# dovidio/jepsen-etcd-demo

Measured on AMD Instinct MI355X. Metric: history ops linearizability-checked/sec (whole node), higher is better.
Workload: dtype u32

## Files before the change

jepsen-etcd-demo_amd/csrc/device_api.hip:

```cpp

#include <dlfcn.h>

#include <atomic>
#include <chrono>
#include <cstring>
#include <functional>
#include <string>
#include <thread>

#include "device_ctx.hpp"

using namespace lcx;

const Rccl *lcx::rccl() {
    static Rccl r;
    static std::once_flag once;
    std::call_once(once, [] {
        void *h = nullptr;
        Dl_info info;
        if (dladdr((void *)&hipStreamCreateWithFlags, &info) && info.dli_fname) {
            std::string dir = info.dli_fname;
            dir = dir.substr(0, dir.find_last_of('/') + 1);
            for (const char *name : {"librccl.so.1", "librccl.so"})
                if (!h) h = dlopen((dir + name).c_str(), RTLD_NOW | RTLD_LOCAL);
// ... 892 lines not shown
        st->total_ms = std::chrono::duration<double, std::milli>(std::chrono::steady_clock::now() - s.t0).count();
        st->lds_keys = c->hctl[2];
        st->wgl_keys = c->hctl[2];
        st->wgl_steps = c->hctl[1];
        st->events = c->hctl[1];
        st->probes = c->hctl[0];
        st->wgl_spilled = ws.wgl_spilled;
    }
    return LC_OK;
}

static int ensure_spec_ws(const Step &s) {
    Dev *c = s.c;
    Lane &L = *s.L;
    LCCHK(grow_dev(c, L.spec_ws, L.spec_ws_words, lcd::spec_ws_words(s.K, s.p.segs)));
    LCCHK(grow_dev(c, L.spec_fin, L.spec_fin_words, s.p.exact ? lcd::spec_fin_words(s.K, s.p.segs) : (size_t)0));
    const int64_t rr_had = L.spec_rr_cap;
    LCCHK(grow_dev(c, L.spec_rr, L.spec_rr_cap, s.K + 2));
    if (L.spec_rr_cap != rr_had) HIPCHK(hipMemsetAsync(L.spec_rr, 0, 2 * sizeof(int32_t), s.q));
    return LC_OK;
}

static int t0_args(Step &s, lcd::Args *a0) {
    Dev *c = s.c;
    if (s.p.t0_step && c->ticket_live && !s.p.competition) {
        s.ticket_base = c->ticket_next;
    } else {
        LCCHK(zero_control(c, s.q));
    }
    c->ticket_live = false;
    if (s.a.n_final && s.K > 0) HIPCHK(hipMemsetAsync(s.a.n_final, 0, (size_t)s.K * 4, s.q));
    const Lists l = lists_of(c);
    *a0 = s.a;
    a0->order = s.d->order; a0->n_order = (int32_t)s.K; a0->n_in = nullptr; a0->ticket = c->counters + 8;
    a0->spill = l.spill0; a0->n_spill = l.n_spill0; a0->wide = l.wide; a0->n_wide = l.n_wide;
    a0->deep = l.spill2; a0->n_deep = l.n_spill2;
    a0->lat_ws = nullptr;
    return LC_OK;
}

static int args_slot(Lane &L, const lcd::Args &a0, lcd::Args **dargs) {
    int aslot = -1;
    for (int q = 0; q < Lane::ARGS_RING && aslot < 0; ++q)
        if (L.args_ok[q] && std::memcmp(L.hargs + q, &a0, sizeof a0) == 0) aslot = q;
    if (aslot < 0) {
        aslot = (int)(L.args_next++ % Lane::ARGS_RING);
        HIPCHK(hipEventSynchronize(L.args_ev[aslot]));
        std::memcpy(L.hargs + aslot, &a0, sizeof a0);
        HIPCHK(hipMemcpyAsync(L.dargs + aslot, L.hargs + aslot, sizeof(lcd::Args), hipMemcpyHostToDevice, L.stream));
        HIPCHK(hipEventRecord(L.args_ev[aslot], L.stream));
        L.args_ok[aslot] = true;
    }
    *dargs = L.dargs + aslot;
    return LC_OK;
}

static lcd::SegArgs seg_args(const Step &s, int grid) {
    Dev *c = s.c;
    const DevBatch *d = s.d;
    const lcd::Args &a = s.a;
    lcd::SegArgs sa{};
    sa.ev_off = d->ev_off; sa.events = d->events; sa.trans = d->trans; sa.key_error = d->key_error;
    sa.n_trans = (uint32_t)d->n_trans; sa.n_keys = (int32_t)s.K; sa.max_seg = lcd::SEG_MAX;
    const double per_key = std::max(1.0, 2.0 * grid / (double)s.K);
    sa.seg_len = (uint32_t)std::max<double>(64.0, (double)d->n_events / (double)s.K / per_key);
    if (c->o->seg_len > 0) sa.seg_len = (uint32_t)c->o->seg_len;
    sa.seg_cnt = c->seg_cnt; sa.seg_end = c->seg_end; sa.seg_out = c->seg_out; sa.seg0_fev = c->seg0_fev;
    sa.work = c->seg_work; sa.rerun = c->seg_rerun; sa.rerun_init = c->seg_rerun_init; sa.ctl = c->seg_ctl;
    sa.err = a.err; sa.valid = a.valid; sa.fail_event = a.fail_event; sa.cause = a.cause;
    sa.rec = a.rec;
    sa.strict = a.strict;
    sa.err_base = a.err_base;
    return sa;
}

static lcd::SpecLaunch spec_launch(const Step &s) {
    Dev *c = s.c;
    const lc_opts &o = *c->o;
    lcd::SpecLaunch l{};
    l.segs = s.p.segs;
    l.ws = s.L->spec_ws; l.rr = s.L->spec_rr; l.parity = s.L->spec_parity;
    l.ck1 = o.spec_ck ? ((uint32_t)o.spec_ck & 0xFFFFu) - 1u : 32u;
    l.ck2 = o.spec_ck ? ((uint32_t)o.spec_ck >> 16) - 1u : 120u;
    l.rerun_grid = c->cu_count;
    l.validate_blocks = s.p.spec_vblocks;
    l.events16 = s.p.ev16 ? s.d->events16 : nullptr;
    l.cost_cuts = (o.path_flags & LC_PATH_SPEC_COST) != 0;
    l.prio = !(o.path_flags & LC_PATH_SPEC_NOPRIO) && !(s.lu && s.lu->overlap);
    l.vfirst = s.p.spec_vfirst;
    l.fin = s.p.exact ? s.L->spec_fin : nullptr;
    l.stage = !(o.path_flags & LC_PATH_SPEC_NOSTAGE);
    return l;
}

static int launch_register_tier(Step &s, const lcd::Args &a0, const lcd::Args *dargs) {
    Dev *c = s.c;
    const lc::StepPlan &p = s.p;
    const int64_t K = s.K;
    if (p.side_validate) {
        HIPCHK(hipEventRecord(c->vin, c->stream));
        HIPCHK(hipStreamWaitEvent(c->stream1, c->vin, 0));
        lcd::Args av = s.a;
        av.n_order = (int32_t)K;
        HIPCHK(lcd::launch_validate(av, c->stream1, p.gen_validate));
        HIPCHK(hipEventRecord(c->vdone, c->stream1));
    }
    if (p.split) {
        const int grid = c->cu_count * 12;
        HIPCHK(hipMemsetAsync(c->seg_ctl, 0, 4 * sizeof(int32_t), c->stream));
        HIPCHK(lcd::launch_segments(seg_args(s, grid), grid, c->stream));
        if (!p.async) HIPCHK(hipEventRecord(c->et0, c->stream));
    } else if (p.spec) {
        HIPCHK(lcd::launch_spec(a0, dargs, spec_launch(s), s.q));
        s.L->spec_parity ^= 1;
        if (!p.async) HIPCHK(hipEventRecord(c->et0, s.q));
    } else if (K > 0 && !s.d->table) {
        HIPCHK(lcd::launch_t0(a0, dargs, p.g0, p.t0_wide, c->stream, s.ticket_base));
        if (!p.async) HIPCHK(hipEventRecord(c->et0, c->stream));
    } else if (K > 0) {
        HIPCHK(hipEventRecord(c->et0, c->stream));
    }
    if (p.side_validate) HIPCHK(hipStreamWaitEvent(c->stream, c->vdone, 0));
    return LC_OK;
}

static void keep_ticket(const Step &s) {
    s.c->ticket_next = (s.p.split || s.p.spec) ? s.ticket_base : s.ticket_base + (uint32_t)s.K + (uint32_t)s.p.g0;
    s.c->ticket_live = true;
}

static int finish_async(const Step &s, lc_stats *st, bool *enqueued) {
    Dev *c = s.c;
    if (s.lu && s.lu->dst) {
        if (s.lu->after) HIPCHK(hipStreamWaitEvent(s.q, s.lu->after, 0));
        HIPCHK(hipMemcpyAsync(s.lu->dst, s.L->rec, s.lu->n * 8, hipMemcpyDeviceToHost, s.q));
    }
    HIPCHK(hipEventRecord(c->ring[c->async_seq % 4], s.q));
    if (s.lu && s.lu->overlap) {
        ++c->run_n;
        c->lane1_live |= s.lu->lane == 1;
    }
    c->ea1_pending = true;
    ++c->async_seq;
    ++c->n_async;
    keep_ticket(s);
    if (st) {
        *st = lc_stats{};
        st->t0_path = s.p.t0_path;
        st->ev_word_bytes = s.p.ev_word_bytes;
    }
    if (enqueued) *enqueued = true;
    return LC_OK;
}

static int run_set_tiers(const Step &s) {
    Dev *c = s.c;
    const Lists l = lists_of(c);
    lcd::Args a1 = s.a;
    a1.order = l.spill0; a1.n_order = 0; a1.n_in = l.n_spill0; a1.ticket = c->counters + 9;
    if (s.d->table) { a1.order = s.d->order; a1.n_order = (int32_t)s.K; a1.n_in = nullptr; }
    a1.spill = l.spill1; a1.n_spill = l.n_spill1; a1.wide = l.wide; a1.n_wide = l.n_wide;
    int g1 = (int)std::min<int64_t>(s.K, (int64_t)c->cu_count * 7);
    HIPCHK(lcd::launch_t1(a1, g1, c->stream));
    lcd::Args a2 = s.a;
    a2.order = l.spill1; a2.n_order = 0; a2.n_in = l.n_spill1; a2.ticket = c->counters + 10;
    a2.spill = l.spill2; a2.n_spill = l.n_spill2; a2.wide = l.wide; a2.n_wide = l.n_wide;
    HIPCHK(lcd::launch_t2(a2, c->cu_count, c->stream));
    return LC_OK;
}

static int read_t0_step(const Step &s) {
// ... 435 lines not shown
```

jepsen-etcd-demo_amd/csrc/device_spec.hip:

```cpp

#include "lattice_core.hpp"
#include "lattice_validate.hpp"

namespace lcd {


constexpr uint32_t SPEC_NONE = 0xFFFFFFFFu;
constexpr uint32_t SPEC_MIN_LEN = 128;
constexpr uint32_t SPEC_MAX_PEND = 6;

template <class EvT>
__device__ __forceinline__ int32_t spec_net(EvT evp, uint32_t b, uint32_t e) {
    constexpr uint32_t G = 8;
    const uint32_t lane = lane_id();
    int32_t cnt = 0;
    for (uint32_t gb = b; gb < e; gb += 64 * G) {
        uint32_t wg[G];
#pragma unroll
        for (uint32_t g = 0; g < G; ++g) {
            const uint32_t j = gb + 64 * g + lane;
            wg[g] = j < e ? evp[j] : 0u;
        }
#pragma unroll
        for (uint32_t g = 0; g < G; ++g) {
// ... 523 lines not shown
__device__ unsigned long long lc_spec_stamps[4096 * 8 * 12];
extern "C" int lc_debug_spec_stamps(unsigned long long *host, int n) {
    return (int)hipMemcpyFromSymbol(host, HIP_SYMBOL(lc_spec_stamps), (size_t)n * 8 * 12 * 8, 0, hipMemcpyDeviceToHost);
}
#define SPEC_STAMP(s, k, v) \
    if (lane == 0 && blk < 4096 && (s) < 8) lc_spec_stamps[((size_t)blk * 8 + (s)) * 12 + (k)] = (v);
#else
#define SPEC_STAMP(s, k, v)
#endif

template <int S, bool E16>
constexpr uint32_t spec_ev_lds() { return (E16 && S > 2) ? (S >= 8 && SPEC_NCK > 2 ? 3072u : 4096u) : 0u; }

#ifndef LC_SPEC2_WAVES
#define LC_SPEC2_WAVES 8
#endif
template <int S, bool E16, bool EX = false>
__global__ __launch_bounds__(64 * S, (S == 2 ? LC_SPEC2_WAVES : S == 8 ? LC_SPEC8_WAVES : 1)) void k_spec(T0Args a) {
#define KA t0k()
    constexpr uint32_t EVC = spec_ev_lds<S, E16>();
    __shared__ uint16_t s_ev[EVC ? EVC : 1];
    __shared__ uint32_t s_end[S][64];
    __shared__ uint32_t s_ck[S][SPEC_NCK][64];
    __shared__ uint32_t s_pend[S][8];
    __shared__ uint64_t s_map[S];
    __shared__ int32_t s_ck_e[S][SPEC_NCK];
    __shared__ int32_t s_cut[S], s_segend[S];
    __shared__ int32_t s_top[S];
    __shared__ int32_t s_ver[S], s_vfev[S];
    __shared__ int32_t s_net[S];
    __shared__ int32_t s_cand[S], s_ncand[S];
    __shared__ int32_t s_prdy[S], s_done[S];
    __shared__ uint32_t s_vx[S][2];
    constexpr bool MEETC = LC_SPEC_MEET && !EX;
    __shared__ int32_t s_meet[MEETC ? S : 1][SPEC_MEET_N];
    constexpr int NWS = spec_lds_ws<S>();
    __shared__ uint32_t s_ws[NWS ? NWS * 3 * T0_RMEM * 64 : 1];
    __shared__ int32_t s_ws_busy[NWS ? NWS : 1];
    const uint32_t lane = lane_id(), wv = uni((uint32_t)threadIdx.x >> 6);
    const uint32_t nb = gridDim.x - (uint32_t)KA.n_order;
    const bool vfirst = (KA.flags & T0_SPEC_VFIRST) != 0;
    const uint32_t blk = vfirst ? blockIdx.x - nb : blockIdx.x;
    if (vfirst ? blockIdx.x < nb : blockIdx.x >= (uint32_t)KA.n_order) {
        const uint32_t vb = vfirst ? blockIdx.x : blockIdx.x - (uint32_t)KA.n_order;
        for (int64_t k = (int64_t)vb * S + wv; k < KA.n_order; k += (int64_t)nb * S) {
            if (EVC > 0 && !(KA.flags & T0_SPEC_NOSTAGE) && KA.ev_off[k + 1] - KA.ev_off[k] <= EVC) continue;
            validate_key<false, E16>(a, k);
        }
        return;
    }
    const int32_t key = (int32_t)uni((uint32_t)KA.order[blk]);
    uint32_t *ws = KA.lat_ws + ((size_t)blk * S + wv) * (3 * T0_RMEM * 64);
    const uint64_t eb = KA.ev_off[key];
    const uint32_t nev = (uint32_t)(KA.ev_off[key + 1] - eb);
    uint32_t n_lds = 0;
    if constexpr (EVC > 0) {
        if (!(KA.flags & T0_SPEC_NOSTAGE)) {
            n_lds = nev < EVC ? nev : EVC;
            const uint16_t *g = KA.events16 + eb;
            for (uint32_t base = 0; base < n_lds; base += 64u * S * 8u) {
                uint16_t v[8];
#pragma unroll
                for (uint32_t q = 0; q < 8; ++q) {
                    const uint32_t j = base + q * 64u * S + threadIdx.x;
                    v[q] = j < n_lds ? g[j] : (uint16_t)0;
                }
#pragma unroll
                for (uint32_t q = 0; q < 8; ++q) {
                    const uint32_t j = base + q * 64u * S + threadIdx.x;
                    if (j < n_lds) s_ev[j] = v[q];
                }
            }
        }
    }
    using EvK = typename std::conditional<(EVC > 0), EvStaged, EvSrc<E16>>::type;
    EvK evp;
    if constexpr (EVC > 0) evp = EvStaged{(LdsU16 *)s_ev, KA.events16 + eb, n_lds};
    else evp = ev_src<E16>(KA) + eb;
    const uint32_t tb = KA.trans_off ? KA.trans_off[key] : 0u;
    const uint32_t ntr = KA.n_trans > tb ? KA.n_trans - tb : 0u;
    const uint32_t *const trp = KA.trans + (ntr ? tb : 0u);
    const uint32_t nstates = KA.trans_off ? (KA.key_states ? KA.key_states[key] : 0xFFFFu) : KA.shared_states;
    const uint32_t width = KA.key_width ? KA.key_width[key] : 0xFFu;
    const bool plain = (KA.key_error && KA.key_error[key]) || nstates > T0_MAX_STATES || nstates == 0 ||
                       width > T0_MAX_WIDTH || KA.init_state >= T0_MAX_STATES || nev < 2 * SPEC_MIN_LEN;
    const uint32_t eff = plain ? 1u : min((uint32_t)S, nev / SPEC_MIN_LEN);
    const uint32_t topmask = nstates >= 32 ? ~0u : (1u << nstates) - 1u;

    if (threadIdx.x < NWS) s_ws_busy[threadIdx.x] = 0;
    if (MEETC && threadIdx.x < S * SPEC_MEET_N) s_meet[threadIdx.x / SPEC_MEET_N][threadIdx.x % SPEC_MEET_N] = -1;
    __syncthreads();
    bool self_val = false;
    uint32_t vc0 = 0, vc1 = 0;
    if constexpr (EVC > 0) {
        self_val = (KA.flags & T0_STRICT) && !(KA.flags & T0_SPEC_NOSTAGE) && n_lds == nev &&
                   !(KA.key_error && KA.key_error[key]);
        const uint32_t nch = (nev + 63u) / 64u;
        vc0 = nch * wv / S;
        vc1 = nch * (wv + 1u) / S;
        if (self_val) {
            uint32_t x0 = 0, x1 = 0;
            for (uint32_t ch = vc0; ch < vc1; ++ch) {
                const uint32_t j = ch * 64u + lane;
                if (j < nev) {
                    const uint32_t sl = LC_EV_SLOT(LC_EV16_WIDE(s_ev[j]));
                    x0 ^= sl < 32u ? 1u << sl : 0u;
                    x1 ^= (sl >= 32u && sl < 64u) ? 1u << (sl - 32u) : 0u;
                }
            }
            x0 = uni(__ockl_wfred_xor_u32(x0));
            x1 = uni(__ockl_wfred_xor_u32(x1));
            if (lane == 0) { s_vx[wv][0] = x0; s_vx[wv][1] = x1; }
        }
    }
    if (wv == 0) {
        for (uint32_t s = 0; s < (uint32_t)S; ++s) { SPEC_STAMP(s, 0, __builtin_amdgcn_s_memtime()) }
    }
    const bool cost = (KA.flags & T0_SPEC_COST) != 0;
    if (!plain && !cost) {
        for (uint32_t p = wv; p + 1 < eff; p += S) {
            const uint32_t t0 = (uint32_t)((uint64_t)nev * p / eff), t1 = (uint32_t)((uint64_t)nev * (p + 1) / eff);
            const int32_t d = spec_net(evp, t0, t1);
            if (lane == 0) s_net[p] = d;
        }
    }
    __syncthreads();
    if constexpr (EVC > 0) {
        if (self_val) {
            const uint32_t vns = KA.trans_off ? (KA.key_states ? KA.key_states[key] : 0u) : KA.shared_states;
            uint32_t pend[2] = {0u, 0u};
            for (uint32_t q = 0; q < wv; ++q) { pend[0] ^= uni(s_vx[q][0]); pend[1] ^= uni(s_vx[q][1]); }
            int32_t why = 0;
            for (uint32_t ch = vc0; ch < vc1 && !why; ++ch) {
                const uint32_t j = ch * 64u + lane;
                const bool in = j < nev;
                const uint32_t w = in ? LC_EV16_WIDE(s_ev[j]) : 0u;
                why = validate_chunk<false, 2>(w, in, trp, ntr, vns, 64u, pend);
            }
            if (why && lane == 0) {
                atomicOr(&KA.err[0], why);
                atomicMax(&KA.err[1], KA.err_base + key + 1);
            }
        }
    }
    if (!plain && !cost) {
        for (uint32_t s = wv; s < eff; s += S) {
            if (s == 0) continue;
            int32_t pend = 0;
            for (uint32_t q = 0; q < s; ++q) pend += uni(s_net[q]);
            const uint32_t t = (uint32_t)((uint64_t)nev * s / eff);
            const uint32_t w = t + lane < nev ? evp[t + lane] : 0u;
            uint32_t n2 = 0;
            const uint32_t c2 = spec_cut_at(w, nev, t, pend, n2);
            if (lane == 0) {
                s_cand[s] = c2 == SPEC_NONE ? -1 : (int32_t)c2;
                s_ncand[s] = (int32_t)n2;
            }
        }
    }
    if (!plain && cost && wv < eff) {
        uint32_t pos_v;
        int32_t pend_v;
        spec_targets_cost(evp, nev, eff, pos_v, pend_v);
        for (uint32_t s = wv; s < eff; s += S) {
            if (s == 0) continue;
            const uint32_t t = uni(__builtin_amdgcn_readlane(pos_v, s));
            const uint32_t w = t + lane < nev ? evp[t + lane] : 0u;
            uint32_t n2 = 0;
            const uint32_t c2 = spec_cut_at(w, nev, t, uni(__builtin_amdgcn_readlane(pend_v, s)), n2);
// ... 46 lines not shown
            if (s == 0) {
                st.W0 = lane == 0 ? 1u << KA.init_state : 0u;
            } else {
                words = spec_pending(evp, cut, n0, np);
                spec_setup(st, words, np, trp, ntr);
                st.W0 = lane < (1u << np) ? topmask : 0u;
            }
            if (lane < 6) s_pend[s][lane] = words;
            if (lane == 6) s_pend[s][6] = np;
            const bool lost = s != 0 && np != n0;
            if (lost && lane == 0) s_top[s] = -3;
            spec_publish(&s_prdy[s]);
            uint32_t fev = 0;
            uint32_t *const sv = EX ? KA.spec_fin + ((size_t)blk * S + s) * 2 * SPEC_SAVE_WORDS : nullptr;
            const int r = lost ? 6
                               : spec_walk<0, NWS, EvK, EX>(evp, trp, ntr, cut, end, st, ws, s_ws, s_ws_busy,
                                                                   s_ck[s], s_ck_e[s], KA.spec_ck1, KA.spec_ck2,
                                                                   fev, !(KA.flags & T0_SPEC_NOPRIO), sv, nullptr,
                                                                   (MEETC && s != 0) ? s_meet[s] : nullptr);
            s_end[s][lane] = st.W0;
            uint64_t map = 0;
            for (uint32_t q = 0; q < 6; ++q) {
                const uint32_t sl = __builtin_amdgcn_readlane(st.slot_v, q);
                if ((st.live >> q) & 1u) map |= (uint64_t)(0x80u | sl) << (8 * q);
            }
            SPEC_STAMP(s, 2, __builtin_amdgcn_s_memtime())
            top_s = r == 1 ? (int32_t)fev : r == 3 ? -2 : r == 6 ? -3 : -1;
            if (lane == 0) {
                s_map[s] = map;
                s_top[s] = top_s;
            }
            spec_publish(&s_done[s]);
        }
        uint32_t v = s + 1;
        while (v < eff && uni(s_cut[v]) < 0) ++v;
        if (kept && top_s == -1 && v < eff) {
            SPEC_STAMP(v, 3, __builtin_amdgcn_s_memtime())
            int32_t ver = 3, vfev = -1;
            uint32_t fev = 0;
            if (spec_wait(&s_prdy[v]) && spec_load(&s_top[v]) != -3) {
                const uint32_t cut = (uint32_t)uni(s_cut[v]), end = (uint32_t)uni(s_segend[v]);
                const uint32_t np = uni(s_pend[v][6]);
                SpecState st{};
                spec_setup(st, lane < 6 ? s_pend[v][lane] : 0u, np, trp, ntr);
                const uint64_t map = uni(s_map[s]);
                uint32_t src = 0;
                for (uint32_t j = 0; j < np; ++j) {
                    const uint32_t sl = __builtin_amdgcn_readlane(st.slot_v, j);
                    uint32_t at = 31;
                    for (uint32_t q = 0; q < 6; ++q)
                        if (((map >> (8 * q)) & 0xFFu) == (0x80u | sl)) at = q;
                    src |= ((lane >> j) & 1u) << at;
                }
                const uint32_t E = (uint32_t)__shfl((int)s_end[s][lane], (int)(src & 63u));
                st.W0 = lane < (1u << np) ? E : 0u;
                uint32_t *const sv =
                    EX ? KA.spec_fin + ((size_t)blk * S + v) * 2 * SPEC_SAVE_WORDS + SPEC_SAVE_WORDS : nullptr;
                const int r = spec_walk<1, NWS, EvK, EX>(evp, trp, ntr, cut, end, st, ws, s_ws, s_ws_busy,
                                                                s_ck[v], s_ck_e[v], 0, 0, fev, false, sv,
                                                                &s_done[v], MEETC ? s_meet[v] : nullptr);
                bool last = true;
                for (uint32_t q = v + 1; q < eff; ++q) last = last && uni(s_cut[q]) < 0;
                if (r == 4) ver = 1;
                else if (r == 1) { ver = 2; vfev = (int32_t)fev; }
                else if (r == 3) ver = 6;
                else if (r == 5) ver = 3;
                else if (last) ver = 5;
                else if (spec_wait(&s_done[v])) ver = (st.n <= 6 && !__any(st.W0 != s_end[v][lane])) ? 1 : 3;
            }
            SPEC_STAMP(v, 7, ((unsigned long long)ver << 32) | (fev - (uint32_t)uni(s_cut[v])))
            SPEC_STAMP(v, 4, __builtin_amdgcn_s_memtime())
            if (lane == 0) {
                s_ver[v] = ver;
                s_vfev[v] = vfev;
            }
        }
    }
    __syncthreads();
    if (wv == 0) {
        for (uint32_t s = 0; s < (uint32_t)S; ++s) { SPEC_STAMP(s, 5, __builtin_amdgcn_s_memtime()) }
    }
    if (wv == 0) {
        const Args &f = *KA.full;
        bool rerun = plain, bad = false;
        int32_t fv = -1;
        uint32_t fin_run = 0;
        if (!plain) {
            for (uint32_t s = 0; s < eff && fv < 0 && !rerun && !bad; ++s) {
                if (uni(s_cut[s]) < 0) continue;
                const int32_t top = uni(s_top[s]);
                if (top == -2) { bad = true; break; }
                if (top == -3) { rerun = true; break; }
                fin_run = 2 * s;
                if (s == 0) { fv = top; continue; }
                const int32_t ver = uni(s_ver[s]);
                if (ver == 1) fv = top;
                else if (ver == 2) { fv = uni(s_vfev[s]); fin_run = 2 * s + 1; }
                else if (ver == 5) fin_run = 2 * s + 1;
                else if (ver == 6) bad = true;
                else rerun = true;
            }
        }
        int kr = K_DONE;
        if (rerun) {
            if (lane == 0) KA.spec_rr[atomicAdd(KA.spec_nrr, 1)] = key;
        } else if (bad) kr = K_SPILL;
        else if (fv >= 0) finish_key(f, key, LC_INVALID, LC_CAUSE_NONLIN, fv, 0, 0, (uint64_t)fv + 1u);
        else finish_key(f, key, LC_VALID, LC_CAUSE_NONE, -1, 0, 0, nev);
        if constexpr (EX) {
            if (!rerun && !bad) {
                uint32_t *const sv = KA.spec_fin + ((size_t)blk * S * 2 + fin_run) * SPEC_SAVE_WORDS;
                const LatMem fm{sv, sv, sv};
                write_final_mem(f, key, fm, lane, sv[T0_RMEM * 64 + lane], uni(sv[(T0_RMEM + 1) * 64]));
            }
        }
        if (kr == K_SPILL) {
            if (KA.flags & T0_STRICT) {
                t0_malformed(KA, key, LC_BATCH_E_FIT);
                finish_key(f, key, LC_UNKNOWN, LC_CAUSE_ERROR, -1, 0, 0, 0);
            } else {
                const bool deep = f.deep && KA.key_width && KA.key_width[key] > LC_DIRECT_T3_WIDTH;
                push_list(deep ? f.deep : f.spill, deep ? f.n_deep : f.n_spill, key, f.list_cap);
            }
        }
    }
}
#undef KA

constexpr int SPEC_RERUN_WAVES = 4;
template <bool E16, bool EX = false>
__global__ __launch_bounds__(64 * SPEC_RERUN_WAVES) void k_spec_rerun(T0Args a) {
    __shared__ uint32_t ws_all[SPEC_RERUN_WAVES][3 * T0_RMEM * 64];
    uint32_t *const ws = ws_all[threadIdx.x >> 6];
    const int32_t n = *a.spec_nrr;
    if (blockIdx.x == 0 && threadIdx.x == 0) *a.spec_nrr_next = 0;
    for (int32_t w = blockIdx.x * SPEC_RERUN_WAVES + (int32_t)(threadIdx.x >> 6); w < n;
         w += gridDim.x * SPEC_RERUN_WAVES) {
        const int32_t key = a.spec_rr[w];
        const int kr = lattice_key<T0_RSMALL, !EX, E16>(a, key, ws);
        if (kr == K_SPILL) t0_spill(a, key);
    }
}

#ifdef LC_T0_COUNT_SWEEPS
int spec_sweep_hist(unsigned long long *host) {
    return (int)hipMemcpyFromSymbol(host, HIP_SYMBOL(lc_sweep_hist), sizeof(lc_sweep_hist), 0, hipMemcpyDeviceToHost);
}
#endif

size_t spec_ws_words(int64_t n_keys, int segs) { return (size_t)std::max<int64_t>(n_keys, 1) * segs * lat_ws_words(); }

size_t spec_fin_words(int64_t n_keys, int segs) {
    return (size_t)std::max<int64_t>(n_keys, 1) * segs * 2 * SPEC_SAVE_WORDS;
}
hipError_t launch_spec(const Args &a, const Args *a_dev, const SpecLaunch &l, hipStream_t s) {
    const int segs = l.segs;
    const uint16_t *const events16 = l.events16;
    uint32_t *const fin = l.fin;
    T0Args t = make_t0(a, a_dev);
    t.events16 = events16;
    if (l.cost_cuts) t.flags |= T0_SPEC_COST;
    if (!l.stage) t.flags |= T0_SPEC_NOSTAGE;
    if (l.vfirst && l.validate_blocks > 0) t.flags |= T0_SPEC_VFIRST;
    if (!l.prio) t.flags |= T0_SPEC_NOPRIO;
    t.lat_ws = l.ws;
    t.spec_ck1 = l.ck1;
    t.spec_ck2 = l.ck2;
    t.spec_nrr = l.rr + (l.parity & 1);
    t.spec_nrr_next = l.rr + ((l.parity & 1) ^ 1);
    t.spec_rr = l.rr + 2;
    t.spec_fin = fin;
    const dim3 grid((unsigned)std::max(1, a.n_order + std::max(0, l.validate_blocks)));
    const dim3 rgrid((unsigned)std::max(1, std::min((a.n_order + SPEC_RERUN_WAVES - 1) / SPEC_RERUN_WAVES, l.rerun_grid)));
#define LC_SPEC_L(SS, E, X) hipLaunchKernelGGL((k_spec<SS, E, X>), grid, dim3(64 * SS), 0, s, t)
#define LC_SPEC_ALL(E)                                      \
    if (fin) {                                              \
        if (segs >= 8) LC_SPEC_L(8, E, true);               \
        else if (segs >= 4) LC_SPEC_L(4, E, true);          \
        else LC_SPEC_L(2, E, true);                         \
    } else if (segs >= 8) LC_SPEC_L(8, E, false);           \
    else if (segs >= 6) LC_SPEC_L(6, E, false);             \
    else if (segs >= 4) LC_SPEC_L(4, E, false);             \
    else if (segs >= 3) LC_SPEC_L(3, E, false);             \
    else LC_SPEC_L(2, E, false);
    if (events16) { LC_SPEC_ALL(true) } else { LC_SPEC_ALL(false) }
#undef LC_SPEC_ALL
#undef LC_SPEC_L
    hipError_t e = hipGetLastError();
    if (e != hipSuccess) return e;
    if (events16) {
        if (fin) hipLaunchKernelGGL((k_spec_rerun<true, true>), rgrid, dim3(64 * SPEC_RERUN_WAVES), 0, s, t);
        else hipLaunchKernelGGL((k_spec_rerun<true, false>), rgrid, dim3(64 * SPEC_RERUN_WAVES), 0, s, t);
    } else {
        if (fin) hipLaunchKernelGGL((k_spec_rerun<false, true>), rgrid, dim3(64 * SPEC_RERUN_WAVES), 0, s, t);
        else hipLaunchKernelGGL((k_spec_rerun<false, false>), rgrid, dim3(64 * SPEC_RERUN_WAVES), 0, s, t);
    }
    return hipGetLastError();
}

}
```

jepsen-etcd-demo_amd/csrc/lattice_core.hpp:

```cpp
#pragma once

#include <hip/hip_runtime.h>

#include <type_traits>

#include <algorithm>
#include <cstdint>

#include "../../include/lincheck.h"
#include "device_common.hpp"
#include "device_search.hpp"
#include "stream_plan.hpp"

extern "C" __device__ uint32_t __ockl_wfred_add_u32(uint32_t);
extern "C" __device__ int32_t __ockl_wfred_add_i32(int32_t);
extern "C" __device__ uint32_t __ockl_wfred_min_u32(uint32_t);
extern "C" __device__ uint32_t __ockl_wfred_xor_u32(uint32_t);

namespace lcd {

constexpr int T0_RSMALL = 4, T0_RBIG = 16;
constexpr int T0_RMEM = 16;
#ifndef LC_T0_MAX_WIDTH
#define LC_T0_MAX_WIDTH 10
// ... 904 lines not shown
    uint32_t W0 = W[0];
    bool dirty = true;
    [[maybe_unused]] bool dense_first = false;
    if constexpr (RESUME) {
        if constexpr (FAST) dirty = rs->dirty;
        dense_first = n >= 7;
    }
    for (uint32_t phase = 0; phase <= nev && e < lim; ++phase) {
        while (e < lim && !(RESUME && dense_first)) {
            T0_PROF_BEGIN
            const uint32_t evi = __builtin_amdgcn_readlane(ev, i);
            const uint32_t slot = LC_EV_SLOT(evi);
            if (!(evi & LC_EV_OK_BIT)) {
                if (n == 6) break;
                if (n >= T0_MAX_WIDTH || slot >= 64) {
                    status = 3;
                } else {
                    const Xfer x{(uint32_t)__builtin_amdgcn_readlane(xc.k, i),
                                 (uint32_t)__builtin_amdgcn_readlane(xc.cap, i),
                                 (uint32_t)__builtin_amdgcn_readlane(xc.b, i)};
                    const uint32_t idx = (uint32_t)__builtin_ctz(~live);
                    slot_v = setl(slot_v, idx, slot);
                    k_v = setl(k_v, idx, x.k);
                    cap_v = setl(cap_v, idx, x.cap);
                    b_v = setl(b_v, idx, x.b);
                    if constexpr (TAG) m_v = setl(m_v, idx, (uint32_t)__builtin_amdgcn_readlane(xc.m, i));
                    dense_v = setl(dense_v, slot, idx);
                    live |= 1u << idx;
                    ++n;
                    dirty = true;
                }
            } else {
                const uint32_t p = __builtin_amdgcn_readlane(dense_v, slot & 63u);
                uint32_t nSn = 0;
                int r;
                if constexpr (FAST && RM == T0_RSMALL) {
                    const uint32_t top = 32u - (uint32_t)__builtin_clz(live);
                    if (top >= 6) r = ok_lane_closed<6, TAG>(W0, p, live, k_v, cap_v, b_v, lane, lm, dirty, m_v);
                    else if (top == 5) r = ok_lane_closed<5, TAG>(W0, p, live, k_v, cap_v, b_v, lane, lm, dirty, m_v);
                    else r = ok_lane_closed<4, TAG>(W0, p, live, k_v, cap_v, b_v, lane, lm, dirty, m_v);
                    dirty = false;
                    k_v = setl(k_v, p, 0u);
                } else {
                const uint32_t pk = __builtin_amdgcn_readlane(k_v, p), pc = __builtin_amdgcn_readlane(cap_v, p),
                               pb = __builtin_amdgcn_readlane(b_v, p);
                k_v = setl(k_v, p, 0u);
                const uint32_t top = 32u - (uint32_t)__builtin_clz(live);
                if (RM == T0_RBIG || top >= 6)
                    r = ok_lane<6>(W0, p, live, k_v, cap_v, b_v, pk, pc, pb, lane, lm, budget, count, probes, nSn,
                                   want_peak);
                else if (top == 5)
                    r = ok_lane<5>(W0, p, live, k_v, cap_v, b_v, pk, pc, pb, lane, lm, budget, count, probes, nSn,
                                   want_peak);
                else
                    r = ok_lane<4>(W0, p, live, k_v, cap_v, b_v, pk, pc, pb, lane, lm, budget, count, probes, nSn,
                                   want_peak);
                }
                live = r ? live : live & ~(1u << p);
                n = r ? n : n - 1;
                peak = nSn > peak ? nSn : peak;
                status = r;
                fev = e;
            }
            T0_PROF_END(evi)
            lim = status ? 0u : lim;
            advance();
        }
        if (e >= lim) break;
        if (!(RESUME && dense_first)) {
            W[0] = W0;
#pragma unroll
            for (int k = 1; k < RM; ++k) W[k] = 0u;
        }
        if constexpr (RESUME) dense_first = false;
        while (e < lim) {
            T0_PROF_BEGIN
            const uint32_t evi = __builtin_amdgcn_readlane(ev, i);
            const uint32_t slot = LC_EV_SLOT(evi);
            if (!(evi & LC_EV_OK_BIT)) {
                if (n >= T0_MAX_WIDTH || slot >= 64) {
                    status = 3;
                } else {
                    if (RM < 16 && n == 8) {
#pragma unroll
                        for (int k = 0; k < T0_RMEM; ++k) m.W[k * 64 + lane] = k < RM ? W[k < RM ? k : 0] : 0u;
                        in_mem = true;
                    }
                    const Xfer x{(uint32_t)__builtin_amdgcn_readlane(xc.k, i),
                                 (uint32_t)__builtin_amdgcn_readlane(xc.cap, i),
                                 (uint32_t)__builtin_amdgcn_readlane(xc.b, i)};
                    const uint32_t idx = n;
                    slot_v = setl(slot_v, idx, slot);
                    k_v = setl(k_v, idx, x.k);
                    cap_v = setl(cap_v, idx, x.cap);
                    b_v = setl(b_v, idx, x.b);
                    if constexpr (TAG) m_v = setl(m_v, idx, (uint32_t)__builtin_amdgcn_readlane(xc.m, i));
                    dense_v = setl(dense_v, slot, idx);
                    live |= 1u << idx;
                    ++n;
                }
            } else {
                const uint32_t p = __builtin_amdgcn_readlane(dense_v, slot & 63u);
                uint32_t nSn = 0;
                int r;
                if (n == 7)
                    r = ok_reg<2, RM, TAG>(W, p, k_v, cap_v, b_v, lane, budget, count, probes, nSn, want_peak, m_v);
                else if (n == 8)
                    r = ok_reg<4, RM, TAG>(W, p, k_v, cap_v, b_v, lane, budget, count, probes, nSn, want_peak, m_v);
                else if constexpr (RM < 16) {
                    if (n == 9)
                        r = ok_event_mem<8, TAG>(m, p, n, k_v, cap_v, b_v, lane, budget, count, probes, nSn, want_peak,
                                                 m_v);
                    else
                        r = ok_event_mem<16, TAG>(m, p, n, k_v, cap_v, b_v, lane, budget, count, probes, nSn, want_peak,
                                                  m_v);
                } else {
                    if (n == 9) r = ok_reg<8>(W, p, k_v, cap_v, b_v, lane, budget, count, probes, nSn, want_peak);
                    else r = ok_reg<16>(W, p, k_v, cap_v, b_v, lane, budget, count, probes, nSn, want_peak);
                }
                const uint32_t last = n - 1;
                const uint32_t s_last = __builtin_amdgcn_readlane(slot_v, last);
                const uint32_t x0 = __builtin_amdgcn_readlane(k_v, last),
                               x1 = __builtin_amdgcn_readlane(cap_v, last), x2 = __builtin_amdgcn_readlane(b_v, last);
                if (!r) {
                    slot_v = setl(slot_v, p, s_last);
                    k_v = setl(k_v, p, x0);
                    cap_v = setl(cap_v, p, x1);
                    b_v = setl(b_v, p, x2);
                    if constexpr (TAG) m_v = setl(m_v, p, (uint32_t)__builtin_amdgcn_readlane(m_v, last));
                    dense_v = setl(dense_v, s_last & 63u, p);
                    k_v = setl(k_v, last, 0u);
                }
                live = r ? live : (1u << last) - 1u;
                if (RM < 16 && in_mem && n == 9 && !r) {
#pragma unroll
                    for (int k = 0; k < RM; ++k) W[k] = m.W[k * 64 + lane];
                    in_mem = false;
                }
                n = r ? n : n - 1;
                peak = nSn > peak ? nSn : peak;
                status = r;
                fev = e;
            }
            T0_PROF_END(evi)
            lim = status ? 0u : lim;
            advance();
            if (n <= 6) break;
        }
        W0 = W[0];
        dirty = true;
    }
#undef T0_PROF_BEGIN
#undef T0_PROF_END
    W[0] = W0;
    out.in_mem = in_mem; out.slot_v = slot_v; out.live = live; out.n = n;
    out.status = status; out.fev = fev; out.peak = peak; out.probes = probes;
    if constexpr (RESUME) {
        rs->in_mem = in_mem;
        rs->k_v = k_v; rs->cap_v = cap_v; rs->b_v = b_v; rs->slot_v = slot_v; rs->dense_v = dense_v;
        rs->n = n; rs->live = live;
        if constexpr (FAST) rs->dirty = dirty;
        else rs->peak = peak;
    }
}

template <int RM, bool FAST, bool E16 = false>
__device__ __forceinline__ int lattice_key(const T0Args &a, int32_t key, uint32_t *ws) {
    const uint32_t lane = lane_id();
    const LatMem m{ws, ws + T0_RMEM * 64, ws + 2 * T0_RMEM * 64};
    const uint64_t eb = a.ev_off[key], ee = a.ev_off[key + 1];
    const uint32_t tb = a.trans_off ? a.trans_off[key] : 0u;
    if (a.key_error && a.key_error[key]) {
        finish_key(*a.full, key, LC_UNKNOWN, LC_CAUSE_ERROR, -1, 0, 0, 0);
        return K_DONE;
    }
    if (a.key_states && a.key_states[key] > LC_WIDE_MAX_STATES) {
        finish_key(*a.full, key, LC_UNKNOWN, LC_CAUSE_STATES, -1, 1, 0, 0);
        return K_DONE;
    }
    const uint32_t nstates = a.trans_off ? (a.key_states ? a.key_states[key] : 0xFFFFu) : a.shared_states;
    const uint32_t width = a.key_width ? a.key_width[key] : 0xFFu;
    if (nstates > T0_MAX_STATES || width > T0_MAX_WIDTH || a.init_state >= T0_MAX_STATES) return K_SPILL;
    const uint64_t budget = FAST ? ~0ull : a.budget;
    const bool want_peak = !FAST && (a.flags & T0_WANT_PEAK) != 0;
    const bool count = !FAST && (a.flags & T0_COUNT) != 0;
    const uint32_t ntr = a.n_trans > tb ? a.n_trans - tb : 0u;
    const uint32_t nev = (a.flags & T0_DBG_NOEVENTS) ? 0u : (uint32_t)(ee - eb);
    uint32_t W[RM];
    LatWalk w;
    lattice_walk<RM, FAST, false>(W, w, ev_src<E16>(a) + eb, nev, a.trans + (ntr ? tb : 0u), ntr, 1u << a.init_state, m,
                                  budget, want_peak, count);
    if (w.status == 3) return K_SPILL;
    const Args &f = *a.full;

    if (!w.in_mem) {
#pragma unroll
        for (int k = 0; k < RM; ++k) m.W[k * 64 + lane] = W[k];
    }
    if (!(a.flags & T0_DBG_NOFINAL)) write_final_mem(f, key, m, lane, w.slot_v, w.live);
    const uint32_t pr = __ockl_wfred_add_u32(w.probes);
    if (w.status)
        finish_key(f, key, w.status == 1 ? LC_INVALID : LC_UNKNOWN,
                   w.status == 1 ? LC_CAUSE_NONLIN : LC_CAUSE_BUDGET, (int32_t)w.fev, w.peak, pr,
                   (uint64_t)w.fev + (w.status == 1 ? 1u : 0u));
    else
        finish_key(f, key, LC_VALID, LC_CAUSE_NONE, -1, w.peak, pr, nev);
    return K_DONE;
}

__device__ __forceinline__ void t0_spill(const T0Args &a, int32_t key) {
    const Args &f = *a.full;
    if (a.flags & T0_STRICT) {
        t0_malformed(a, key, LC_BATCH_E_FIT);
        finish_key(f, key, LC_UNKNOWN, LC_CAUSE_ERROR, -1, 0, 0, 0);
    } else {
        const bool deep = f.deep && a.key_width && a.key_width[key] > LC_DIRECT_T3_WIDTH;
        push_list(deep ? f.deep : f.spill, deep ? f.n_deep : f.n_spill, key, f.list_cap);
    }
}

static T0Args make_t0(const Args &a, const Args *a_dev) {
    T0Args t{};
    t.ev_off = a.ev_off; t.events = a.events; t.trans = a.trans; t.trans_off = a.trans_off;
    t.key_width = a.key_width; t.key_states = a.key_states; t.key_error = a.key_error; t.order = a.order;
    t.ticket = a.ticket;
    t.err = a.err;
    t.err_base = a.err_base;
    t.n_trans = a.n_trans;
    t.lat_ws = a.lat_ws; t.full = a_dev; t.budget = a.budget; t.n_order = a.n_order;
    t.init_state = a.init_state; t.shared_states = a.shared_states;
    t.flags = (a.count_probes ? T0_COUNT : 0u) | (a.peak ? T0_WANT_PEAK : 0u) | (a.final_cfg ? T0_WANT_FINAL : 0u) |
              (a.debug_mode == 2 ? T0_DBG_NOEVENTS : 0u) | (a.debug_mode == 3 ? T0_DBG_NOFINAL : 0u) |
              (a.strict ? T0_STRICT : 0u);
    return t;
}

}
```

jepsen-etcd-demo_amd/csrc/step_plan.hpp:

```cpp
#pragma once

#include <algorithm>
#include <cstdint>

#include "../../include/lincheck.h"

namespace lc {

struct StepIn {
    int64_t K = 0;
    uint64_t n_events = 0;
    int cu_count = 256;
    bool t0_only = false, table = false, taggable = false, seg_pays = false, validated = false, has_events16 = false;
    int32_t algorithm = LC_ALGO_LINEAR, flags = 0, path_flags = 0, spec_segs = 0;
    uint64_t max_configs = 1ull << 20;
    bool want_peak = false, want_final = false, want_n_final = false;
    bool res_host = false;
    bool allow_async = false;
    int spec8_waves = 8;
    uint64_t ws_words = 0, fin_words = 0;
    uint64_t ws_max_bytes = 8ull << 30;
};

struct StepPlan {
    bool wgl_only = false;
    bool competition = false;
    bool t0_step = false;
    bool async = false;
    bool split = false;
    bool spec = false;
    int segs = 0;
    bool exact = false;
    bool ev16 = false;
    bool t0_wide = false;
    int g0 = 1;
    bool strict = false;
    bool gen_validate = false;
    bool side_validate = false;
    int spec_vblocks = 0;
    bool spec_vfirst = false;
    uint32_t t0_path = LC_T0_PATH_NONE;
    uint32_t ev_word_bytes = 0;
};

inline StepPlan plan_step(const StepIn &in) {
    StepPlan p;
    const int64_t K = in.K;
    p.strict = !in.validated && in.t0_only;
    p.gen_validate = !in.validated && !in.t0_only;
    if (in.algorithm == LC_ALGO_WGL) {
        p.wgl_only = true;
        return p;
    }
    p.competition = in.algorithm == LC_ALGO_COMPETITION;
    p.t0_step = K > 0 && in.t0_only && !(in.flags & LC_OPT_COUNT_PROBES);
    p.async = p.t0_step && in.allow_async && !p.competition && !in.res_host;
    const bool fast = !in.want_peak && !in.want_final && in.max_configs >= 16ull * 64 * 32;
    const bool want = (in.path_flags & LC_PATH_SPLIT_ON) ? true : (in.path_flags & LC_PATH_SPLIT_OFF) ? false : in.seg_pays;
    p.split = p.t0_step && fast && in.taggable && want && K <= (int64_t)in.cu_count * 8;
    int segs = K > 0 ? (int)std::min<int64_t>(8, (int64_t)in.cu_count * 4 * 4 / std::max<int64_t>(K, 1)) : 0;
    segs = segs >= 8 ? 8 : segs >= 4 ? 4 : K > 0 ? 2 : 0;
    const bool exact_spec = !in.want_peak && in.want_final && in.want_n_final && in.max_configs >= 16ull * 64 * 32;
    if (in.spec8_waves >= 8 && (fast || exact_spec) && K > 0 && K * 8 <= (int64_t)in.cu_count * 4 * 8) segs = 8;
    if (in.spec_segs) segs = in.spec_segs;
    p.exact = exact_spec && !fast;
    if (p.exact) segs = segs >= 8 ? 8 : segs >= 4 ? 4 : 2;
    p.segs = segs;
    p.spec = !p.split && p.t0_step && (fast || exact_spec) && segs >= 2 && !(in.path_flags & LC_PATH_SPEC_OFF);
    if (p.spec && (uint64_t)K * (uint64_t)segs * (in.ws_words + (p.exact ? in.fin_words : 0)) * 4 > in.ws_max_bytes)
        p.spec = false;
    p.ev16 = p.spec && in.has_events16;
    p.t0_path = K == 0 || in.table ? LC_T0_PATH_NONE
                : p.split          ? LC_T0_PATH_SEGMENTS
                : p.spec           ? LC_T0_PATH_SPEC
                                   : LC_T0_PATH_LATTICE;
    p.ev_word_bytes = p.t0_path ? (p.ev16 ? 2u : 4u) : 0u;
    p.t0_wide = K <= (int64_t)in.cu_count * 8;
    p.g0 = (int)std::max<int64_t>(1, std::min<int64_t>(K, (int64_t)in.cu_count * (p.t0_wide ? 8 : 16)));
    p.side_validate = K > 0 && ((p.strict && !p.spec) || p.gen_validate);
    p.spec_vblocks = p.spec && p.strict ? (int)std::min<int64_t>(K, in.cu_count) : 0;
    p.spec_vfirst = p.spec && K * segs > (int64_t)in.cu_count * 16;
    return p;
}

}
```

Baseline: 6.260 billion.

## Rework spec rerun kernel to single-wave blocks with global workspace and small grid

The speculative rerun kernel moves from four waves per block with per-wave LDS workspace to one wave per block using a slice of the global lattice workspace. Its grid becomes a small planned value, capped at eight and at K. Plain keys (errors, too many states) are now finished or spilled directly instead of being queued for rerun, and lattice memory writes use a lane-permuted address. The aim is to avoid rerun queue traffic and LDS pressure, at the cost of much less rerun parallelism and global-memory rather than LDS workspace access.

```diff
diff --git a/jepsen-etcd-demo_amd/csrc/device_api.hip b/jepsen-etcd-demo_amd/csrc/device_api.hip
--- a/jepsen-etcd-demo_amd/csrc/device_api.hip
+++ b/jepsen-etcd-demo_amd/csrc/device_api.hip
@@ -998,11 +998,14 @@
     l.ws = s.L->spec_ws; l.rr = s.L->spec_rr; l.parity = s.L->spec_parity;
     l.ck1 = o.spec_ck ? ((uint32_t)o.spec_ck & 0xFFFFu) - 1u : 32u;
     l.ck2 = o.spec_ck ? ((uint32_t)o.spec_ck >> 16) - 1u : 120u;
-    l.rerun_grid = c->cu_count;
+    l.rerun_grid = s.p.rerun_grid;
     l.validate_blocks = s.p.spec_vblocks;
     l.events16 = s.p.ev16 ? s.d->events16 : nullptr;
     l.cost_cuts = (o.path_flags & LC_PATH_SPEC_COST) != 0;
-    l.prio = !(o.path_flags & LC_PATH_SPEC_NOPRIO) && !(s.lu && s.lu->overlap);
+#ifndef LC_SPEC_PRIO_OVERLAP
+#define LC_SPEC_PRIO_OVERLAP 0
+#endif
+    l.prio = !(o.path_flags & LC_PATH_SPEC_NOPRIO) && (LC_SPEC_PRIO_OVERLAP || !(s.lu && s.lu->overlap));
     l.vfirst = s.p.spec_vfirst;
     l.fin = s.p.exact ? s.L->spec_fin : nullptr;
     l.stage = !(o.path_flags & LC_PATH_SPEC_NOSTAGE);
diff --git a/jepsen-etcd-demo_amd/csrc/device_spec.hip b/jepsen-etcd-demo_amd/csrc/device_spec.hip
--- a/jepsen-etcd-demo_amd/csrc/device_spec.hip
+++ b/jepsen-etcd-demo_amd/csrc/device_spec.hip
@@ -629,9 +629,11 @@
     const uint32_t *const trp = KA.trans + (ntr ? tb : 0u);
     const uint32_t nstates = KA.trans_off ? (KA.key_states ? KA.key_states[key] : 0xFFFFu) : KA.shared_states;
     const uint32_t width = KA.key_width ? KA.key_width[key] : 0xFFu;
-    const bool plain = (KA.key_error && KA.key_error[key]) || nstates > T0_MAX_STATES || nstates == 0 ||
-                       width > T0_MAX_WIDTH || KA.init_state >= T0_MAX_STATES || nev < 2 * SPEC_MIN_LEN;
-    const uint32_t eff = plain ? 1u : min((uint32_t)S, nev / SPEC_MIN_LEN);
+    const bool plain = (KA.key_error && KA.key_error[key]) ||
+                       (KA.key_states && KA.key_states[key] > LC_WIDE_MAX_STATES) || nstates > T0_MAX_STATES ||
+                       width > T0_MAX_WIDTH || KA.init_state >= T0_MAX_STATES;
+    const bool whole = plain || nstates == 0 || nev < 2 * SPEC_MIN_LEN;
+    const uint32_t eff = whole ? 1u : min((uint32_t)S, nev / SPEC_MIN_LEN);
     const uint32_t topmask = nstates >= 32 ? ~0u : (1u << nstates) - 1u;
 
     if (threadIdx.x < NWS) s_ws_busy[threadIdx.x] = 0;
@@ -844,7 +846,7 @@
     }
     if (wv == 0) {
         const Args &f = *KA.full;
-        bool rerun = plain, bad = false;
+        bool rerun = false, bad = false;
         int32_t fv = -1;
         uint32_t fin_run = 0;
         if (!plain) {
@@ -864,13 +866,18 @@
             }
         }
         int kr = K_DONE;
-        if (rerun) {
+        if (plain) {
+            if (KA.key_error && KA.key_error[key]) finish_key(f, key, LC_UNKNOWN, LC_CAUSE_ERROR, -1, 0, 0, 0);
+            else if (KA.key_states && KA.key_states[key] > LC_WIDE_MAX_STATES)
+                finish_key(f, key, LC_UNKNOWN, LC_CAUSE_STATES, -1, 1, 0, 0);
+            else kr = K_SPILL;
+        } else if (rerun) {
             if (lane == 0) KA.spec_rr[atomicAdd(KA.spec_nrr, 1)] = key;
         } else if (bad) kr = K_SPILL;
         else if (fv >= 0) finish_key(f, key, LC_INVALID, LC_CAUSE_NONLIN, fv, 0, 0, (uint64_t)fv + 1u);
         else finish_key(f, key, LC_VALID, LC_CAUSE_NONE, -1, 0, 0, nev);
         if constexpr (EX) {
-            if (!rerun && !bad) {
+            if (!plain && !rerun && !bad) {
                 uint32_t *const sv = KA.spec_fin + ((size_t)blk * S * 2 + fin_run) * SPEC_SAVE_WORDS;
                 const LatMem fm{sv, sv, sv};
                 write_final_mem(f, key, fm, lane, sv[T0_RMEM * 64 + lane], uni(sv[(T0_RMEM + 1) * 64]));
@@ -889,15 +896,12 @@
 }
 #undef KA
 
-constexpr int SPEC_RERUN_WAVES = 4;
 template <bool E16, bool EX = false>
-__global__ __launch_bounds__(64 * SPEC_RERUN_WAVES) void k_spec_rerun(T0Args a) {
-    __shared__ uint32_t ws_all[SPEC_RERUN_WAVES][3 * T0_RMEM * 64];
-    uint32_t *const ws = ws_all[threadIdx.x >> 6];
+__global__ __launch_bounds__(64) void k_spec_rerun(T0Args a) {
+    uint32_t *const ws = a.lat_ws + (size_t)blockIdx.x * (3 * T0_RMEM * 64);
     const int32_t n = *a.spec_nrr;
     if (blockIdx.x == 0 && threadIdx.x == 0) *a.spec_nrr_next = 0;
-    for (int32_t w = blockIdx.x * SPEC_RERUN_WAVES + (int32_t)(threadIdx.x >> 6); w < n;
-         w += gridDim.x * SPEC_RERUN_WAVES) {
+    for (int32_t w = (int32_t)blockIdx.x; w < n; w += (int32_t)gridDim.x) {
         const int32_t key = a.spec_rr[w];
         const int kr = lattice_key<T0_RSMALL, !EX, E16>(a, key, ws);
         if (kr == K_SPILL) t0_spill(a, key);
@@ -933,7 +937,7 @@
     t.spec_rr = l.rr + 2;
     t.spec_fin = fin;
     const dim3 grid((unsigned)std::max(1, a.n_order + std::max(0, l.validate_blocks)));
-    const dim3 rgrid((unsigned)std::max(1, std::min((a.n_order + SPEC_RERUN_WAVES - 1) / SPEC_RERUN_WAVES, l.rerun_grid)));
+    const dim3 rgrid((unsigned)std::max(1, std::min(a.n_order * segs, l.rerun_grid)));
 #define LC_SPEC_L(SS, E, X) hipLaunchKernelGGL((k_spec<SS, E, X>), grid, dim3(64 * SS), 0, s, t)
 #define LC_SPEC_ALL(E)                                      \
     if (fin) {                                              \
@@ -951,11 +955,11 @@
     hipError_t e = hipGetLastError();
     if (e != hipSuccess) return e;
     if (events16) {
-        if (fin) hipLaunchKernelGGL((k_spec_rerun<true, true>), rgrid, dim3(64 * SPEC_RERUN_WAVES), 0, s, t);
-        else hipLaunchKernelGGL((k_spec_rerun<true, false>), rgrid, dim3(64 * SPEC_RERUN_WAVES), 0, s, t);
+        if (fin) hipLaunchKernelGGL((k_spec_rerun<true, true>), rgrid, dim3(64), 0, s, t);
+        else hipLaunchKernelGGL((k_spec_rerun<true, false>), rgrid, dim3(64), 0, s, t);
     } else {
-        if (fin) hipLaunchKernelGGL((k_spec_rerun<false, true>), rgrid, dim3(64 * SPEC_RERUN_WAVES), 0, s, t);
-        else hipLaunchKernelGGL((k_spec_rerun<false, false>), rgrid, dim3(64 * SPEC_RERUN_WAVES), 0, s, t);
+        if (fin) hipLaunchKernelGGL((k_spec_rerun<false, true>), rgrid, dim3(64), 0, s, t);
+        else hipLaunchKernelGGL((k_spec_rerun<false, false>), rgrid, dim3(64), 0, s, t);
     }
     return hipGetLastError();
 }
diff --git a/jepsen-etcd-demo_amd/csrc/lattice_core.hpp b/jepsen-etcd-demo_amd/csrc/lattice_core.hpp
--- a/jepsen-etcd-demo_amd/csrc/lattice_core.hpp
+++ b/jepsen-etcd-demo_amd/csrc/lattice_core.hpp
@@ -1010,8 +1010,9 @@
                     status = 3;
                 } else {
                     if (RM < 16 && n == 8) {
-#pragma unroll
-                        for (int k = 0; k < T0_RMEM; ++k) m.W[k * 64 + lane] = k < RM ? W[k < RM ? k : 0] : 0u;
+                        uint32_t *const mW = m.W + opq_lane(lane);
+#pragma unroll
+                        for (int k = 0; k < T0_RMEM; ++k) mW[k * 64] = k < RM ? W[k < RM ? k : 0] : 0u;
                         in_mem = true;
                     }
                     const Xfer x{(uint32_t)__builtin_amdgcn_readlane(xc.k, i),
@@ -1061,8 +1062,9 @@
                 }
                 live = r ? live : (1u << last) - 1u;
                 if (RM < 16 && in_mem && n == 9 && !r) {
-#pragma unroll
-                    for (int k = 0; k < RM; ++k) W[k] = m.W[k * 64 + lane];
+                    const uint32_t *const mW = m.W + opq_lane(lane);
+#pragma unroll
+                    for (int k = 0; k < RM; ++k) W[k] = mW[k * 64];
                     in_mem = false;
                 }
                 n = r ? n : n - 1;
@@ -1122,8 +1124,9 @@
     const Args &f = *a.full;
 
     if (!w.in_mem) {
-#pragma unroll
-        for (int k = 0; k < RM; ++k) m.W[k * 64 + lane] = W[k];
+        uint32_t *const mW = m.W + opq_lane(lane);
+#pragma unroll
+        for (int k = 0; k < RM; ++k) mW[k * 64] = W[k];
     }
     if (!(a.flags & T0_DBG_NOFINAL)) write_final_mem(f, key, m, lane, w.slot_v, w.live);
     const uint32_t pr = __ockl_wfred_add_u32(w.probes);
diff --git a/jepsen-etcd-demo_amd/csrc/step_plan.hpp b/jepsen-etcd-demo_amd/csrc/step_plan.hpp
--- a/jepsen-etcd-demo_amd/csrc/step_plan.hpp
+++ b/jepsen-etcd-demo_amd/csrc/step_plan.hpp
@@ -39,9 +39,15 @@
     bool side_validate = false;
     int spec_vblocks = 0;
     bool spec_vfirst = false;
+    int rerun_grid = 1;
     uint32_t t0_path = LC_T0_PATH_NONE;
     uint32_t ev_word_bytes = 0;
 };
+
+#ifndef LC_SPEC_RERUN_GRID
+#define LC_SPEC_RERUN_GRID 8
+#endif
+constexpr int SPEC_RERUN_GRID = LC_SPEC_RERUN_GRID;
 
 inline StepPlan plan_step(const StepIn &in) {
     StepPlan p;
@@ -80,6 +86,7 @@
     p.side_validate = K > 0 && ((p.strict && !p.spec) || p.gen_validate);
     p.spec_vblocks = p.spec && p.strict ? (int)std::min<int64_t>(K, in.cu_count) : 0;
     p.spec_vfirst = p.spec && K * segs > (int64_t)in.cu_count * 16;
+    p.rerun_grid = (int)std::max<int64_t>(1, std::min<int64_t>(SPEC_RERUN_GRID, p.spec ? K : 1));
     return p;
 }
 
```

Measured after the change: 6.560 billion (median of 6 runs). 4.8% higher.
